# supersimple33/aruco-slam

Measured on AMD Instinct MI355X. Metric: EKF updates/sec at n=1024 landmarks, m=32 obs/frame, higher is better.
Workload: dtype f32 covariance / f64 state

## Files before the change

aruco_slam_amd/csrc/ekf_api.hip:

```cpp
#include <atomic>
#include <cstring>

#include "ekf_host.h"
#include "ekf_kernels.h"

thread_local std::string g_err;

namespace {

std::atomic<ekf_filter*> g_pipelining{nullptr};

void release_pipelining_token(ekf_filter* f) { (void)g_pipelining.compare_exchange_strong(f, nullptr); }

constexpr int kStageSlots = 64;
constexpr int kMacroSuper = 8;
constexpr int kMacroMinTiles = 3000;
constexpr int kTimedKernels = 4;
constexpr int kWideVisible = 1024;
inline int visible_cap(int model) { return model == EKF_MODEL_ROTATIONS ? 50 : 64; }
inline bool wide_frame(int model, int m) { return m > visible_cap(model); }
constexpr int kEventPool = 2048;

struct Layout {
    int64_t cap;
// ... 39 lines not shown
    L.has_cov2 = c.cov_kernel != EKF_COVK_VALU && (c.flags & 5) == 0;
    L.off_cov2 = L.has_cov2 ? w.take((size_t)L.cap * L.cap * L.elem) : 0;
    L.off_wdbg = w.take((size_t)L.kmax * L.cap * 8);
    L.off_idx = w.take((size_t)c.max_visible * 4);
    L.off_z = w.take((size_t)c.max_visible * 7 * 8);
    L.off_status = w.take(256);
    L.off_stamps = w.take(64 * 8);
    L.off_dx = w.take((size_t)L.cap * 8);
    L.off_diag = w.take((size_t)L.cap * 8);
    L.off_xyz = w.take((size_t)256 * 6 * 8);
    L.off_unc = w.take((size_t)256 * 10 * 8);
    {
        const size_t nb = (size_t)L.kmax / EKF_RB;
        L.xl_dop = nb * (nb - 1) / 2 * 256 + 64;
        L.xl_y = L.xl_dop + nb * 256;
        L.xl_jac = L.xl_y + L.kmax;
        L.xl_tag = L.xl_jac + (size_t)L.kmax * EKF_JLD;
        L.xl_xs = L.xl_tag + 32;
        L.xl_xr = L.xl_xs + nb * (nb + 1) / 2 * 256;
        L.xl_stag = L.xl_xr + (size_t)round_up(L.kmax, 16);
        L.xl_len = L.xl_stag + 256;
        L.off_xl = w.take(2 * L.xl_len * 8);
        L.off_done = w.take(256);
        L.off_sync = w.take(256);
        L.wsup_ld = (int)round_up(EKF_CAM + (int64_t)L.lmd * c.max_visible, 32);
        L.off_wsup = w.take((size_t)2 * L.kmax * L.wsup_ld * L.elem);
    }
    {
        const int tmax = (int)(L.cap / 128);
        L.tiles_cap = (L.elem == 4 && c.cov_kernel != EKF_COVK_VALU && c.cov_kernel != EKF_COVK_MFMA_TILE)
                          ? tmax * (tmax + 1) / 2 + 8 * kMacroSuper * kMacroSuper : 0;
        L.off_tiles = w.take((size_t)L.tiles_cap * 4);
    }
    L.off_wwork = wide ? w.take((size_t)L.kmax * L.cap * 8) : 0;
    L.off_xinv = wide ? w.take((size_t)EKF_WIDE_BLOCK * EKF_WIDE_BLOCK * 8) : 0;
    L.total = w.end;
    L.slot_bytes = std::max(align256((size_t)c.max_visible * 4) + align256((size_t)c.max_visible * 56),
                            align256(256 * 48) + align256(256 * 80));
    return L;
}

int check_config(const ekf_config* c) {
    if (!c) return fail(EKF_ERR_INVALID, "config is NULL");
    if (c->max_landmarks < 1) return fail(EKF_ERR_INVALID, "max_landmarks must be >= 1");
    if (c->model != EKF_MODEL_EKF && c->model != EKF_MODEL_ROTATIONS)
        return fail(EKF_ERR_INVALID, "unknown model");
    if (c->max_visible < 1 || c->max_visible > ((c->flags & EKF_FLAG_WIDE_FRAMES) ? kWideVisible : visible_cap(c->model)))
// ... 29 lines not shown
};

struct ekf_filter {
    ekf_config cfg{};
    Layout lay{};
    hipStream_t stream = nullptr;
    hipStream_t big = nullptr;
    hipEvent_t ev_front = nullptr;
    GetterShortcut shortcut;
    int device = 0;
    void* cov = nullptr;
    int64_t ld = 0;
    double* state = nullptr;
    char* ws = nullptr;
    bool bound = false, is_reset = false;
    int n_lm = 0;
    int last_m = 0;
    bool debug_w = false;
    bool debug_stamps = false;
    bool debug_stamps_light = false;
    uint64_t fseq = 0;
    uint64_t done_total = 0;
    uint64_t la_base = 0;
    int la_ok = -1;
    int seq_mode = EKF_SEQ_NONE;
    int tiles_T = -1, tiles_grid = 0;
    PinnedBuffer ring, readback, tiles_host;
    int slot = 0;
    hipEvent_t slot_done[kStageSlots] = {};
    bool timing = false;
    bool timing_cov_only = false;
    std::vector<hipEvent_t> ev;
    int ev_frames = 0;
    double t_sum_us[kTimedKernels] = {};
    int64_t t_cnt[kTimedKernels] = {};
    PinnedBuffer log_pin[2];
    hipEvent_t log_pin_done[2] = {};
    int log_pin_turn = 0;
    int64_t log_stats[4] = {};

    int dims() const { return lay.lmd * n_lm + EKF_CAM; }
    template <typename P> P* at(size_t off) const { return reinterpret_cast<P*>(ws + off); }
};

namespace {

// ... 286 lines not shown
}

struct RunFrame {
    const int32_t* idx;
    const double* z;
    int m;
    double* traj_row;
};

template <class FrameAt>
int run_pipelined(ekf_filter* f, int frames, FrameAt frame_at, void* other) {
    const Layout& L = f->lay;
    int rc = ensure_tiles(f);
    if (rc) return rc;
    void* wbuf[2] = {f->at<void>(L.off_wpanel), f->at<void>(L.off_wpanel2)};
    void* cbuf[2] = {f->cov, other};
    char* wsup0 = f->at<char>(L.off_wsup);
    void* wsup[2] = {wsup0, wsup0 + (size_t)L.kmax * L.wsup_ld * L.elem};
    unsigned long long* sync = f->at<unsigned long long>(L.off_sync);
    int32_t* status = f->at<int32_t>(L.off_status);
    const uint64_t base = f->la_base;
    f->shortcut.run();
    RunFrame nx = frame_at(0);
    for (int t = 0; t < frames; ++t) {
        const int par = t & 1;
        const RunFrame cf_t = nx;
        EkfFrame fr = make_frame(f, cf_t.idx, cf_t.z, cf_t.m, cf_t.traj_row);
        fr.cov = cbuf[0];
        fr.wpanel = wbuf[par];
        if (t > 0) {
            fr.cov = cbuf[par ^ 1];
            fr.wprev = wbuf[par ^ 1];
            fr.wsup_prev = wsup[par ^ 1];
        }
        const int nb = fr.kpad / EKF_RB;
        const int grid = nb * (nb + 1) / 2 + 2 + fr.ncols / 64;
        fr.wsup_ld = L.wsup_ld;
        fr.la_sync = sync;
        fr.la_signal = (t > 0) ? base + (uint64_t)t : 0;
        fr.la_gate = (t > 0) ? base + (uint64_t)t : 0;
        fr.lds_min = grid <= 100 ? 148 * 1024 : 0;
        if (t + 1 < frames) {
            nx = frame_at(t + 1);
            fr.next_idx = nx.idx;
            fr.next_m = nx.m;
            fr.wsup = wsup[par];
        }
        bind_exchange(f, fr);
        by_cov_type(f, [&](auto elem) { ekf_launch_front<decltype(elem)>(fr, f->stream); });
        EkfFrame cu = fr;
        cu.cov = cbuf[par];
        cu.cov_out = cbuf[par ^ 1];
        if (t + 1 < frames) {
            ekf_launch_gate(sync, base + (uint64_t)t + 1, status, f->big);
            by_cov_type(f, [&](auto elem) { ekf_launch_cov_update<decltype(elem)>(cu, 2, f->big); });
            ekf_launch_signal(sync + 1, base + (uint64_t)t + 1, f->big);
        } else {
            by_cov_type(f, [&](auto elem) { ekf_launch_cov_update<decltype(elem)>(cu, 2, f->stream); });
        }
        HIP_TRY(hipGetLastError());
        f->last_m = cf_t.m;
    }
    f->cov = cbuf[frames & 1];
    f->la_base = base + (uint64_t)frames;
    return EKF_OK;
}

struct RunPlan {
    std::vector<char> candidate;
    std::vector<char> joins;
    bool want_runs = false;
};

template <class MOf, class NNewOf>
RunPlan plan_runs(const ekf_filter* f, int frames, MOf m_of, NNewOf nnew_of) {
    RunPlan p;
    p.candidate.assign((size_t)frames, 0);
    p.joins.assign((size_t)frames, 0);
    int prev_kpad = -1;
// ... 70 lines not shown
}

int open_handle(ekf_filter* f) {
    int rc = reserve_host_buffers(f, f->lay);
    if (rc) return rc;
    HIP_TRY(hipStreamCreateWithFlags(&f->big, hipStreamNonBlocking));
    HIP_TRY(hipEventCreateWithFlags(&f->ev_front, hipEventDisableTiming));
    for (hipEvent_t& e : f->slot_done) HIP_TRY(hipEventCreateWithFlags(&e, hipEventDisableTiming));
    return EKF_OK;
}

int clear_buffers(const ekf_filter* f, void* cov, double* state, char* ws, const Layout& L) {
    HIP_TRY(hipMemsetAsync(cov, 0, (size_t)L.cap * L.cap * L.elem, f->stream));
    HIP_TRY(hipMemsetAsync(state, 0, (size_t)L.cap * 8, f->stream));
    HIP_TRY(hipMemsetAsync(ws, 0, L.total, f->stream));
    HIP_TRY(hipMemsetD32Async(reinterpret_cast<hipDeviceptr_t>(ws + L.off_xl), (int)0xFFFBADC0u, L.xl_len * 4, f->stream));
    return EKF_OK;
}

void restart_workspace(ekf_filter* f) {
    f->fseq = 0;
    f->done_total = 0;
    f->la_base = 0;
    f->tiles_T = -1;
    std::memset(f->readback.get(), 0, 256 + (size_t)f->lay.cap * 8);
}

}

extern "C" {

const char* ekf_last_error_string(void) { return g_err.c_str(); }

int ekf_default_config(ekf_config* cfg) {
    if (!cfg) return fail(EKF_ERR_INVALID, "config is NULL");
    std::memset(cfg, 0, sizeof(*cfg));
    cfg->max_landmarks = 50;
    cfg->max_visible = 50;
    cfg->cov_dtype = EKF_COV_F64;
    cfg->quat_mode = EKF_QUAT_AS_WRITTEN;
    cfg->cov_kernel = EKF_COVK_AUTO;
    cfg->model = EKF_MODEL_EKF;
    cfg->initial_camera_uncertainty = 0.1;
    cfg->initial_landmark_uncertainty = 0.7;
    cfg->r_uncertainty = 0.9;
    cfg->q_cam = 0.3;
// ... 603 lines not shown
```

aruco_slam_amd/csrc/ekf_cov_macro.hip:

```cpp
#include <hip/hip_ext.h>
#include "ekf_kernels.h"

typedef float cm_f32x16 __attribute__((ext_vector_type(16)));
typedef float cm_f4 __attribute__((ext_vector_type(4)));

#define CM_NW 8
#define CM_T (64 * CM_NW)
#define CM_LD 132
#define CM_KC 16
#define CM_NBUF 5
#define CM_LDS_BYTES (CM_NBUF * 2 * CM_KC * 128 * 4)

#define CM_MID 0
#define CM_STAGGER 24000

__device__ __forceinline__ void cm_store16(float* p, const cm_f4& v) {
    asm volatile("global_store_dwordx4 %0, %1, off sc1\n\ts_nop 1" ::"v"(p), "v"(v) : "memory");
}

__device__ __forceinline__ void cm_dma16(const float* g, float* lds_wave_base) {
    __builtin_amdgcn_global_load_lds((const __attribute__((address_space(1))) void*)g,
                                     (__attribute__((address_space(3))) void*)lds_wave_base, 16, 0, 0);
}

// ... 13 lines not shown
        if (ch == target) seen = true;
    }
    for (int i = 0; i < steps; ++i) {
        if (i + depth < nch) {
            if (seen) n += dpw;
            if (i + depth == target) seen = true;
        }
        if (i < npb && seen) n += 16;
    }
    return n;
}
template <int N> __device__ __forceinline__ void cm_wait_vm() { asm volatile("s_waitcnt vmcnt(%0)" ::"n"(N) : "memory"); }

template <int KB, int NW>
__global__ __launch_bounds__(64 * NW) __attribute__((amdgpu_waves_per_eu(NW / 2, NW / 2)))
void ekf_cov_update_macro_f32(EkfFrame fr, const uint32_t* __restrict__ tiles) {
    extern __shared__ __attribute__((aligned(16))) float cm_sm[];
    constexpr int NT = 64 * NW, WC = NW / 2, CW = 128 / WC, TJ = CW / 32;
    constexpr int DPW = 16 / NW;
    constexpr int NPB = 2 * TJ;
    constexpr int DEPTH = CM_NBUF - 1;
    static_assert(NW == 8, "wait counts below are worked out for 8 waves");
    const uint32_t tl = tiles[blockIdx.x];
    if (tl == 0xFFFFFFFFu) return;
    const int I = (int)(tl >> 16), J = (int)(tl & 0xFFFFu);
    const int tid = threadIdx.x, lane = tid & 63, l31 = lane & 31, lhi = lane >> 5;
    const int wave = __builtin_amdgcn_readfirstlane(tid >> 6);
    const int wr = wave / WC, wc = wave % WC;
    const int i0 = 128 * I, j0 = 128 * J;
    const float* __restrict__ wp = static_cast<const float*>(fr.wpanel);
    const float* __restrict__ P = static_cast<const float*>(fr.cov);
    float* Pout = fr.cov_out ? static_cast<float*>(fr.cov_out) : static_cast<float*>(fr.cov);
    const int ld = (int)fr.ld, ldw = (int)fr.ldw;
    constexpr int NCH = KB;

    if (blockIdx.x < 512 && ((__builtin_amdgcn_s_getreg((31 << 11) | 4) / (NW / 4)) & 1)) {
        const long long t0 = __builtin_amdgcn_s_memtime();
        while (__builtin_amdgcn_s_memtime() - t0 < CM_STAGGER) __builtin_amdgcn_s_sleep(32);
    }
    const unsigned wlane = (unsigned)(lhi * ldw + 4 * l31);
    auto stage = [&](int c) {
        float* buf = cm_sm + (c % CM_NBUF) * (2 * CM_KC * 128);
        const int rloc = 2 * wave;
        const float* src = wp + (int64_t)(CM_KC * c + rloc) * ldw;
        cm_dma16(src + i0 + wlane, buf + rloc * 128);
        cm_dma16(src + j0 + wlane, buf + CM_KC * 128 + rloc * 128);
    };
// ... 107 lines not shown
        for (int it = 0; it < NPASS; ++it) cm_store16(ob + (int64_t)(RPP * it) * ld + (unsigned)(prow * ld + pcol), rowv[it]);
    }
    if (!dtile) __syncthreads();
    if (!dtile) {
#pragma unroll
    for (int ti = 0; ti < 2; ++ti)
#pragma unroll
        for (int tj = 0; tj < TJ; ++tj)
#pragma unroll
            for (int rg = 0; rg < 4; ++rg) {
                const cm_f4 v = {acc[ti][tj][4 * rg], acc[ti][tj][4 * rg + 1], acc[ti][tj][4 * rg + 2], acc[ti][tj][4 * rg + 3]};
                *reinterpret_cast<cm_f4*>(img + (CW * wc + 32 * tj + l31) * CM_LD + 64 * wr + 32 * ti + 8 * rg + 4 * lhi) = v;
            }
    __syncthreads();
    {
        cm_f4 rowv[NPASS];
#pragma unroll
        for (int it = 0; it < NPASS; ++it) rowv[it] = *reinterpret_cast<const cm_f4*>(img + (RPP * it + prow) * CM_LD + pcol);
        float* ob = Pout + (int64_t)j0 * ld + i0;
#pragma unroll
        for (int it = 0; it < NPASS; ++it) cm_store16(ob + (int64_t)(RPP * it) * ld + (unsigned)(prow * ld + pcol), rowv[it]);
    }
    }
}

int ekf_cov_macro_table(int T, int S, uint32_t* out, int capacity) {
    struct Sup { int si, sj, count; };
    const int NS = (T + S - 1) / S;
    Sup sup[4096];
    int nsup = 0;
    for (int si = 0; si < NS; ++si)
        for (int sj = 0; sj <= si; ++sj) {
            int cnt = 0;
            for (int I = si * S; I < T && I < (si + 1) * S; ++I)
                for (int J = sj * S; J < T && J < (sj + 1) * S && J <= I; ++J) ++cnt;
            if (cnt > 0 && nsup < 4096) sup[nsup++] = Sup{si, sj, cnt};
        }
    for (int a = 1; a < nsup; ++a) {
        const Sup x = sup[a];
        int b = a - 1;
        while (b >= 0 && sup[b].count < x.count) { sup[b + 1] = sup[b]; --b; }
        sup[b + 1] = x;
    }
    int load[8] = {0, 0, 0, 0, 0, 0, 0, 0};
    int owner[4096];
    for (int a = 0; a < nsup; ++a) {
        int x = 0;
        for (int q = 1; q < 8; ++q)
            if (load[q] < load[x]) x = q;
        owner[a] = x;
        load[x] += sup[a].count;
    }
    int maxlen = 0;
    for (int q = 0; q < 8; ++q) maxlen = load[q] > maxlen ? load[q] : maxlen;
    const int grid = 8 * maxlen;
    if (!out) return grid;
    if (grid > capacity) return -1;
    for (int b = 0; b < grid; ++b) out[b] = 0xFFFFFFFFu;
    int pos[8] = {0, 0, 0, 0, 0, 0, 0, 0};
    for (int a = 0; a < nsup; ++a) {
        const int x = owner[a];
        for (int I = sup[a].si * S; I < T && I < (sup[a].si + 1) * S; ++I)
            for (int J = sup[a].sj * S; J < T && J < (sup[a].sj + 1) * S && J <= I; ++J)
                out[8 * (pos[x]++) + x] = ((uint32_t)I << 16) | (uint32_t)J;
    }
    return grid;
}

template <int KB>
static void cm_go(const EkfFrame& fr, hipStream_t s, hipEvent_t e0, hipEvent_t e1) {
    static bool once = false;
    if (!once) {
        (void)hipFuncSetAttribute(reinterpret_cast<const void*>(&ekf_cov_update_macro_f32<KB, CM_NW>),
                                  hipFuncAttributeMaxDynamicSharedMemorySize, CM_LDS_BYTES);
        once = true;
    }
    if (e0) hipExtLaunchKernelGGL((ekf_cov_update_macro_f32<KB, CM_NW>), dim3(fr.cov_grid), dim3(CM_T), CM_LDS_BYTES, s, e0, e1, 0, fr, fr.cov_tiles);
    else hipLaunchKernelGGL((ekf_cov_update_macro_f32<KB, CM_NW>), dim3(fr.cov_grid), dim3(CM_T), CM_LDS_BYTES, s, fr, fr.cov_tiles);
}

void ekf_launch_cov_update_macro(const EkfFrame& fr, hipStream_t s, hipEvent_t e0, hipEvent_t e1) {
    switch (fr.kpad / 16) {
#define CM_CASE(KB) case KB: return cm_go<KB>(fr, s, e0, e1);
        CM_CASE(1) CM_CASE(2) CM_CASE(3) CM_CASE(4) CM_CASE(5) CM_CASE(6) CM_CASE(7) CM_CASE(8) CM_CASE(9) CM_CASE(10)
        CM_CASE(11) CM_CASE(12) CM_CASE(13) CM_CASE(14) CM_CASE(15) CM_CASE(16) CM_CASE(17) CM_CASE(18) CM_CASE(19)
        CM_CASE(20) CM_CASE(21) CM_CASE(22) CM_CASE(23) CM_CASE(24)
#undef CM_CASE
        default: return;
    }
}
```

aruco_slam_amd/csrc/ekf_cov_update.hip:

```cpp
#include <hip/hip_ext.h>
#include "ekf_kernels.h"

template <typename T>
__device__ __forceinline__ void ekf_cov_store(T* p, T v) {
    __hip_atomic_store(p, v, __ATOMIC_RELAXED, __HIP_MEMORY_SCOPE_AGENT);
}

typedef float f32x16 __attribute__((ext_vector_type(16)));
typedef double f64x4 __attribute__((ext_vector_type(4)));

template <typename T>
__global__ __launch_bounds__(256) void ekf_cov_update_valu(EkfFrame fr) {
    __shared__ T sa[16][64];
    __shared__ T sb[16][64];
    const int tid = threadIdx.x, tx = tid & 15, ty = tid >> 4;
    const int i0 = blockIdx.y * 64, j0 = blockIdx.x * 64;
    const T* __restrict__ wp = static_cast<const T*>(fr.wpanel);
    T acc[4][4];
#pragma unroll
    for (int x = 0; x < 4; ++x)
#pragma unroll
        for (int y = 0; y < 4; ++y) acc[x][y] = (T)0;
    for (int kc = 0; kc < fr.kpad; kc += 16) {
#pragma unroll
// ... 19 lines not shown
    }
    T* __restrict__ P = static_cast<T*>(fr.cov);
#pragma unroll
    for (int x = 0; x < 4; ++x) {
        const int row = i0 + ty * 4 + x;
#pragma unroll
        for (int y = 0; y < 4; ++y) {
            const int col = j0 + tx * 4 + y;
            T v = P[(int64_t)row * fr.ld + col];
            if (row == col) v += (T)ekf_qdiag(row, fr.dims, fr.nz);
            P[(int64_t)row * fr.ld + col] = v + acc[x][y];
        }
    }
}

__device__ __forceinline__ void ekf_tri_decode(int item, int& I, int& J) {
    int i = (int)((sqrtf(8.0f * (float)item + 1.0f) - 1.0f) * 0.5f);
    while (i * (i + 1) / 2 > item) --i;
    while ((i + 1) * (i + 2) / 2 <= item) ++i;
    I = i;
    J = item - i * (i + 1) / 2;
}

template <int KB, int DMAX = 3, int WPE = 5>
__global__ __launch_bounds__(256) __attribute__((amdgpu_waves_per_eu(WPE, WPE)))
void ekf_cov_update_mfma_f32(EkfFrame fr, int nitems) {
    __shared__ float tr[4][32][33];
    const int wave = threadIdx.x >> 6, lane = threadIdx.x & 63;
    const int l31 = lane & 31, lhi = lane >> 5;
    const int item = __builtin_amdgcn_readfirstlane(blockIdx.x * 4 + wave);
    if (item >= nitems) return;
    int I, J;
    ekf_tri_decode(item, I, J);
    const int i0 = 32 * I, j0 = 32 * J;
    const float* __restrict__ wp = static_cast<const float*>(fr.wpanel);
    const float* __restrict__ P = static_cast<const float*>(fr.cov);
    float* Pout = fr.cov_out ? static_cast<float*>(fr.cov_out) : static_cast<float*>(fr.cov);
    const int ld = (int)fr.ld, ldw = (int)fr.ldw;
    constexpr int NCH = KB, D = (NCH < DMAX) ? NCH : DMAX;
    float ra[D][8], rb[D][8], pt[16];
    const unsigned wlane = 4u * (unsigned)(lhi * ldw + l31);
    const unsigned plane = 4u * (unsigned)(4 * lhi * ld + l31);
    const uint64_t kstep = 8ull * (uint64_t)ldw;
    uint64_t ua = reinterpret_cast<uint64_t>(wp + i0), ub = reinterpret_cast<uint64_t>(wp + j0);
    const float* __restrict__ ptile = P + (int64_t)i0 * ld + j0;
    float* otile = Pout + (int64_t)i0 * ld + j0;
#define EKF_GLD(dst, voff, sbase) asm volatile("global_load_dword %0, %1, %2" : "=v"(dst) : "v"(voff), "s"(sbase) : "memory")
#define EKF_WAIT16(n, A, B)                                                                              \
    asm volatile("s_waitcnt vmcnt(%16)"                                                                   \
                 : "+v"(A[0]), "+v"(A[1]), "+v"(A[2]), "+v"(A[3]), "+v"(A[4]), "+v"(A[5]), "+v"(A[6]), "+v"(A[7]), \
// ... 29 lines not shown
            case 0: EKF_WAIT16(0, ra[c % D], rb[c % D]); break;
            case 16: EKF_WAIT16(16, ra[c % D], rb[c % D]); break;
            case 32: EKF_WAIT16(32, ra[c % D], rb[c % D]); break;
            case 48: EKF_WAIT16(48, ra[c % D], rb[c % D]); break;
            default: EKF_WAIT16(63, ra[c % D], rb[c % D]); break;
        }
#pragma unroll
        for (int u = 0; u < 8; ++u)
            acc = __builtin_amdgcn_mfma_f32_32x32x2f32(-ra[c % D][u], rb[c % D][u], acc, 0, 0, 0);
        __builtin_amdgcn_sched_barrier(0);
        if (c + D < NCH) {
#pragma unroll
            for (int u = 0; u < 8; ++u) {
                EKF_GLD(ra[c % D][u], wlane, ua);
                EKF_GLD(rb[c % D][u], wlane, ub);
                ua += kstep;
                ub += kstep;
            }
        }
        __builtin_amdgcn_sched_barrier(0);
    }
    asm volatile("s_waitcnt vmcnt(0)"
                 : "+v"(pt[0]), "+v"(pt[1]), "+v"(pt[2]), "+v"(pt[3]), "+v"(pt[4]), "+v"(pt[5]), "+v"(pt[6]), "+v"(pt[7]),
                   "+v"(pt[8]), "+v"(pt[9]), "+v"(pt[10]), "+v"(pt[11]), "+v"(pt[12]), "+v"(pt[13]), "+v"(pt[14]), "+v"(pt[15]));
#undef EKF_GLD
#undef EKF_WAIT16
    const float qlane = (I == J) ? (float)ekf_qdiag(i0 + l31, fr.dims, fr.nz) : 0.0f;
    float out[16];
    auto stf = [](float* base, unsigned off, float v) { ekf_cov_store(reinterpret_cast<float*>(reinterpret_cast<char*>(base) + off), v); };
#pragma unroll
    for (int reg = 0; reg < 16; ++reg) {
        const int rl = (reg & 3) + 8 * (reg >> 2) + 4 * lhi;
        const float v = (pt[reg] + ((rl == l31) ? qlane : 0.0f)) + acc[reg];
        out[reg] = v;
        stf(otile + (int64_t)((reg & 3) + 8 * (reg >> 2)) * ld, plane, v);
    }
    if (I != J) {
#pragma unroll
        for (int reg = 0; reg < 16; ++reg)
            tr[wave][(reg & 3) + 8 * (reg >> 2) + 4 * lhi][l31] = out[reg];
        __builtin_amdgcn_wave_barrier();
        float* pm = Pout + (int64_t)j0 * ld + i0;
        const unsigned mlane = 4u * (unsigned)(lhi * ld + l31);
#pragma unroll
        for (int it = 0; it < 16; ++it)
            stf(pm + (int64_t)(2 * it) * ld, mlane, tr[wave][l31][2 * it + lhi]);
    }
}

__global__ __launch_bounds__(256) void ekf_cov_update_mfma_f64(EkfFrame fr, int nitems) {
    __shared__ double tr[4][32][33];
    const int wave = threadIdx.x >> 6, lane = threadIdx.x & 63;
    const int c = lane & 15, g = lane >> 4;
    const int item = blockIdx.x * 4 + wave;
    if (item >= nitems) return;
    int I, J;
    ekf_tri_decode(item, I, J);
    const int i0 = 32 * I, j0 = 32 * J;
    const double* __restrict__ wp = static_cast<const double*>(fr.wpanel);
    const double* P = static_cast<const double*>(fr.cov);
    double* Pout = fr.cov_out ? static_cast<double*>(fr.cov_out) : static_cast<double*>(fr.cov);
    const int64_t ld = fr.ld, ldw = fr.ldw;

    double pt[2][2][4];
#pragma unroll
    for (int ri = 0; ri < 2; ++ri)
#pragma unroll
        for (int ci = 0; ci < 2; ++ci)
#pragma unroll
            for (int r = 0; r < 4; ++r)
                pt[ri][ci][r] = P[(int64_t)(i0 + 16 * ri + g + 4 * r) * ld + j0 + 16 * ci + c];
    f64x4 acc[2][2];
#pragma unroll
    for (int ri = 0; ri < 2; ++ri)
// ... 15 lines not shown
            b1[u] = wb[off + 16];
        }
#pragma unroll
        for (int u = 0; u < 4; ++u) {
            acc[0][0] = __builtin_amdgcn_mfma_f64_16x16x4f64(-a0[u], b0[u], acc[0][0], 0, 0, 0);
            acc[0][1] = __builtin_amdgcn_mfma_f64_16x16x4f64(-a0[u], b1[u], acc[0][1], 0, 0, 0);
            acc[1][0] = __builtin_amdgcn_mfma_f64_16x16x4f64(-a1[u], b0[u], acc[1][0], 0, 0, 0);
            acc[1][1] = __builtin_amdgcn_mfma_f64_16x16x4f64(-a1[u], b1[u], acc[1][1], 0, 0, 0);
        }
    }
#pragma unroll
    for (int ri = 0; ri < 2; ++ri)
#pragma unroll
        for (int ci = 0; ci < 2; ++ci)
#pragma unroll
            for (int r = 0; r < 4; ++r) {
                const int rl = 16 * ri + g + 4 * r, cl = 16 * ci + c;
                double v = pt[ri][ci][r];
                if (I == J && rl == cl) v += ekf_qdiag(i0 + rl, fr.dims, fr.nz);
                v += acc[ri][ci][r];
                ekf_cov_store(Pout + (int64_t)(i0 + rl) * ld + j0 + cl, v);
                if (I != J) tr[wave][rl][cl] = v;
            }
    if (I != J) {
        __builtin_amdgcn_wave_barrier();
        const int l31 = lane & 31, lhi = lane >> 5;
#pragma unroll
        for (int it = 0; it < 16; ++it) {
            const int cc = 2 * it + lhi;
            ekf_cov_store(Pout + (int64_t)(j0 + cc) * ld + i0 + l31, tr[wave][l31][cc]);
        }
    }
}

__global__ __launch_bounds__(256) void ekf_cov_update_mfma_f64_split(EkfFrame fr, int nitems) {
    __shared__ double tr[32][33];
    const int wave = threadIdx.x >> 6, lane = threadIdx.x & 63;
    const int c = lane & 15, g = lane >> 4;
    const int ri = wave >> 1, ci = wave & 1;
    int I, J;
    ekf_tri_decode(blockIdx.x, I, J);
    const int i0 = 32 * I, j0 = 32 * J;
    const double* __restrict__ wp = static_cast<const double*>(fr.wpanel);
    const double* P = static_cast<const double*>(fr.cov);
    double* Pout = fr.cov_out ? static_cast<double*>(fr.cov_out) : static_cast<double*>(fr.cov);
    const int64_t ld = fr.ld, ldw = fr.ldw;
    double pt[4];
#pragma unroll
    for (int r = 0; r < 4; ++r) pt[r] = P[(int64_t)(i0 + 16 * ri + g + 4 * r) * ld + j0 + 16 * ci + c];
    f64x4 acc = {0.0, 0.0, 0.0, 0.0};
    const double* wa = wp + (int64_t)g * ldw + i0 + 16 * ri + c;
    const double* wb = wp + (int64_t)g * ldw + j0 + 16 * ci + c;
    const int steps = fr.kpad >> 2;
    for (int ks = 0; ks < steps; ks += 4) {
        double a[4], b[4];
#pragma unroll
        for (int u = 0; u < 4; ++u) {
            const int64_t off = (int64_t)(4 * (ks + u)) * ldw;
            a[u] = wa[off];
            b[u] = wb[off];
        }
#pragma unroll
        for (int u = 0; u < 4; ++u) acc = __builtin_amdgcn_mfma_f64_16x16x4f64(-a[u], b[u], acc, 0, 0, 0);
    }
#pragma unroll
    for (int r = 0; r < 4; ++r) {
        const int rl = 16 * ri + g + 4 * r, cl = 16 * ci + c;
        double v = pt[r];
        if (I == J && rl == cl) v += ekf_qdiag(i0 + rl, fr.dims, fr.nz);
        v += acc[r];
        ekf_cov_store(Pout + (int64_t)(i0 + rl) * ld + j0 + cl, v);
        if (I != J) tr[rl][cl] = v;
    }
    if (I != J) {
        __syncthreads();
        const int l31 = threadIdx.x & 31;
        for (int cc = threadIdx.x >> 5; cc < 32; cc += 8)
            ekf_cov_store(Pout + (int64_t)(j0 + cc) * ld + i0 + l31, tr[l31][cc]);
    }
}

__global__ void ekf_gate_kernel(unsigned long long* counter, unsigned long long target, int32_t* status, int max_polls) {
    if (threadIdx.x != 0) return;
    int it = 0;
    while (__hip_atomic_load(counter, __ATOMIC_RELAXED, __HIP_MEMORY_SCOPE_SYSTEM) < target) {
        if (++it > max_polls) { atomicOr(status, EKF_ST_GATE_TIMEOUT); break; }
        __builtin_amdgcn_s_sleep(8);
    }
}
__global__ void ekf_signal_kernel(unsigned long long* counter, unsigned long long value) {
    if (threadIdx.x == 0) __hip_atomic_store(counter, value, __ATOMIC_RELAXED, __HIP_MEMORY_SCOPE_SYSTEM);
}
void ekf_launch_gate(unsigned long long* counter, unsigned long long target, int32_t* status, hipStream_t s, int max_polls) {
    hipLaunchKernelGGL(ekf_gate_kernel, dim3(1), dim3(64), 0, s, counter, target, status, max_polls);
}
void ekf_launch_signal(unsigned long long* counter, unsigned long long value, hipStream_t s) {
    hipLaunchKernelGGL(ekf_signal_kernel, dim3(1), dim3(64), 0, s, counter, value);
}

#define EKF_COV_LAUNCH(kernel, grid, block, s, e0, e1, ...)                                     \
    do {                                                                                         \
        if (e0) hipExtLaunchKernelGGL(kernel, grid, block, 0, s, e0, e1, 0, __VA_ARGS__);        \
        else hipLaunchKernelGGL(kernel, grid, block, 0, s, __VA_ARGS__);                         \
    } while (0)

static inline int ekf_tri_items(const EkfFrame& fr) {
    const int t = (fr.dims + 31) / 32;
    return t * (t + 1) / 2;
}

template <>
void ekf_launch_cov_update<float>(const EkfFrame& fr, int variant, hipStream_t s, hipEvent_t e0, hipEvent_t e1) {
    if (variant == 1) {
        EKF_COV_LAUNCH(ekf_cov_update_valu<float>, dim3(fr.ncols / 64, fr.ncols / 64), dim3(256), s, e0, e1, fr);
    } else if (fr.cov_tiles) {
        ekf_launch_cov_update_macro(fr, s, e0, e1);
    } else {
        const int items = ekf_tri_items(fr);
        const dim3 grid((items + 3) / 4), block(256);
        switch (fr.kpad / 16) {
#define EKF_COV_CASE(KB) case KB: EKF_COV_LAUNCH((ekf_cov_update_mfma_f32<KB, 3, (KB <= 8) ? 5 : 4>), grid, block, s, e0, e1, fr, items); break;
            EKF_COV_CASE(1) EKF_COV_CASE(2) EKF_COV_CASE(3) EKF_COV_CASE(4) EKF_COV_CASE(5) EKF_COV_CASE(6)
            EKF_COV_CASE(7) EKF_COV_CASE(8) EKF_COV_CASE(9) EKF_COV_CASE(10) EKF_COV_CASE(11) EKF_COV_CASE(12)
            EKF_COV_CASE(13) EKF_COV_CASE(14) EKF_COV_CASE(15) EKF_COV_CASE(16) EKF_COV_CASE(17) EKF_COV_CASE(18)
            EKF_COV_CASE(19) EKF_COV_CASE(20) EKF_COV_CASE(21) EKF_COV_CASE(22) EKF_COV_CASE(23) EKF_COV_CASE(24)
            default: break;
#undef EKF_COV_CASE
        }
    }
}
template <>
void ekf_launch_cov_update<double>(const EkfFrame& fr, int variant, hipStream_t s, hipEvent_t e0, hipEvent_t e1) {
    if (variant == 1) {
        EKF_COV_LAUNCH(ekf_cov_update_valu<double>, dim3(fr.ncols / 64, fr.ncols / 64), dim3(256), s, e0, e1, fr);
    } else {
        const int items = ekf_tri_items(fr);
        if (items <= 2048)
            EKF_COV_LAUNCH(ekf_cov_update_mfma_f64_split, dim3(items), dim3(256), s, e0, e1, fr, items);
        else
            EKF_COV_LAUNCH(ekf_cov_update_mfma_f64, dim3((items + 3) / 4), dim3(256), s, e0, e1, fr, items);
    }
}
```

aruco_slam_amd/csrc/ekf_front_impl.h:

```cpp
#pragma once
#include "ekf_solve_big.h"

#define FR_T 512
#define FR_ALD 66
#define FR_KS 96
#define FR_KS64 48
__host__ __device__ inline size_t fr_chunk_a_len(int kpad, bool fix, int elem) {
    const size_t a = (size_t)kpad * FR_ALD;
    const size_t st = elem == 4 ? (size_t)(FR_KS * 128 + FR_KS * 64 + 128 * 64) / 2 : (size_t)(2 * FR_KS64 * 64 + 64 * 64);
    return (fix && a < st) ? st : a;
}
#define FR_SLOTS 4

typedef double pf64x4 __attribute__((ext_vector_type(4)));
template <typename T>
__device__ __forceinline__ void fr_w_store(T* p, T v) {
    __hip_atomic_store(p, v, __ATOMIC_RELAXED, __HIP_MEMORY_SCOPE_AGENT);
}
typedef float fr_f32x16 __attribute__((ext_vector_type(16)));

__device__ __forceinline__ void ekf_poll_sleep() { __builtin_amdgcn_s_sleep(4); }

template <int MODEL>
__device__ __forceinline__ void fr_measure(const EkfFrame& fr, const double* cam, const int* lmc, double* hs,
// ... 212 lines not shown
    int* lmc = reinterpret_cast<int*>(rsd + fr.kpad);
    const int tid = threadIdx.x;
    if (fr.stamps && !fr.stamps_heavy && tid == 0) fr.stamps[16 + ((long long)fr.seqno & 15)] = wall_clock64();
    if (fr.la_signal && tid == 0)
        __hip_atomic_store(fr.la_sync, fr.la_signal, __ATOMIC_RELAXED, __HIP_MEMORY_SCOPE_SYSTEM);
    double cam[EKF_CAM];
#pragma unroll
    for (int a = 0; a < EKF_CAM; ++a) cam[a] = fr.state[a];
    if (tid < fr.m) lmc[tid] = ekf_lm_column(fr, LMD, tid, true);
    __syncthreads();
    fr_measure<MODEL>(fr, cam, lmc, hs, rsd, tid, true);
    __syncthreads();
    double* __restrict__ xj = fr.xl + fr.xl_jac;
    const int nel = fr.k * JC;
    for (int e = tid; e < nel; e += FR_T) ekf_stc(xj + e, hs[e]);
    for (int e = tid; e < fr.kpad; e += FR_T) ekf_stc(fr.xr + e, rsd[e]);
    if (tid == 0) {
        ekf_stc(fr.xl + fr.xl_tag, fr.seqno);
        ekf_stc(fr.xl + fr.xl_tag + 16, fr.seqno);
    }
    if (fr.stamps && tid == 0) fr.stamps[55] = wall_clock64();
    if (fr.la_gate && tid == 0) {
        int it = 0;
        while (__hip_atomic_load(fr.la_sync + 1, __ATOMIC_RELAXED, __HIP_MEMORY_SCOPE_SYSTEM) < fr.la_gate) {
            if (++it > (1 << 22)) { ekf_raise(fr, EKF_ST_GATE_TIMEOUT); break; }
            __builtin_amdgcn_s_sleep(8);
        }
    }
}

__device__ __forceinline__ int fr_tag_stale(double tag, double seqno) { return !ekf_is_sent(tag) && tag != seqno; }
struct SvIoFused {
    const EkfFrame& fr;
    int spin_fail, stale;
    __device__ __forceinline__ bool settled(const sf64x4& v) const {
        return !__any(ekf_is_sent(v[0]) || ekf_is_sent(v[1]) || ekf_is_sent(v[2]) || ekf_is_sent(v[3]));
    }
    __device__ __forceinline__ void settle_block(sf64x4& v, int i, int tc, int lane) {
        const double* base = fr.xs + sv_blk_index(i, tc);
        int it = 0;
        while (!settled(v)) {
            if (++it > EKF_SPIN_MAX) { spin_fail = 1; break; }
            ekf_poll_sleep();
            v = sf64x4{ekf_ldc(base + 2 * lane), ekf_ldc(base + 2 * lane + 1), ekf_ldc(base + 128 + 2 * lane),
                       ekf_ldc(base + 129 + 2 * lane)};
        }
    }
    __device__ __forceinline__ sf64x4 fetch_resid(int tc, int g) {
        const double* base = fr.xr + EKF_RB * tc + g;
        sf64x4 v = {ekf_ldc(base), ekf_ldc(base + 4), ekf_ldc(base + 8), ekf_ldc(base + 12)};
        int it = 0;
// ... 864 lines not shown
```

aruco_slam_amd/csrc/ekf_kernels.h:

```cpp
#pragma once
#include <hip/hip_runtime.h>
#include <stdint.h>
#include "ekf_device.h"

#define EKF_ST_NOT_SPD 1
#define EKF_ST_TIMEOUT 4
#define EKF_ST_STALE_JAC 16
#define EKF_ST_STALE_COL 32
#define EKF_ST_STALE_S 64
#define EKF_ST_BAD_INDEX 128
#define EKF_ST_GATE_TIMEOUT 256

struct EkfFrame {
    void* cov;
    int64_t ld;
    double* state;
    int32_t model;
    int32_t dims;
    int32_t ncols;
    int32_t m;
    int32_t k;
    int32_t kpad;
    const int32_t* idx;
    const double* z;
// ... 5 lines not shown
    double* sblk;
    int32_t sblk_rows;
    double* lmat;
    int32_t ldl;
    double* dinv;
    double* lop;
    double* dop;
    double* yvec;
    void* wpanel;
    int64_t ldw;
    double* wdbg;
    int32_t* status;
    double* traj_row;
    double* dxvec;
    long long* stamps;
    int32_t stamps_heavy;
    const int32_t* next_idx;
    int32_t next_m;
    void* cov_out;
    const void* wprev;
    const void* wsup_prev;
    unsigned long long* la_sync;
    unsigned long long la_signal, la_gate;
    int32_t lds_min;
    void* wsup;
    int32_t wsup_ld;
    EkfNoise nz;
    int32_t quat_mode;
    double* xl;
    double* xl_next;
    int32_t xl_dop, xl_y, xl_jac;
    int32_t xl_len;
    double* xs;
    double* xr;
    double* xs_tag;
    int32_t n_lm;
    unsigned long long* done_ctr;
    unsigned long long done_target;
    int32_t xl_tag;
    double seqno;
    double* state_host;
    int32_t* status_host;
    const uint32_t* cov_tiles;
    int32_t cov_grid;
};

__device__ __forceinline__ void ekf_raise(const EkfFrame& fr, int bits) {
    atomicOr(fr.status, bits);
    if (fr.status_host) __hip_atomic_store(fr.status_host, 1, __ATOMIC_RELAXED, __HIP_MEMORY_SCOPE_SYSTEM);
}

__device__ __forceinline__ int ekf_lm_column(const EkfFrame& fr, int lmd, int j, bool flag) {
    int i = fr.idx[j];
    if ((unsigned)i >= (unsigned)fr.n_lm) {
        if (flag) ekf_raise(fr, EKF_ST_BAD_INDEX);
        i = 0;
    }
    return EKF_CAM + lmd * i;
}

__device__ inline void ekf_inject_camera(const EkfFrame& fr, const double err[3], const double x[3]) {
    double q[4] = {fr.state[3], fr.state[4], fr.state[5], fr.state[6]};
    ekf_quat_inject(q, err, fr.quat_mode);
    for (int i = 0; i < 4; ++i) fr.state[3 + i] = q[i];
    for (int i = 0; i < 3; ++i) fr.state[7 + i] = 0.0;
    if (fr.traj_row) {
        fr.traj_row[0] = x[0]; fr.traj_row[1] = x[1]; fr.traj_row[2] = x[2];
        for (int i = 0; i < 4; ++i) fr.traj_row[3 + i] = q[i];
    }
}

template <typename T> void ekf_launch_front(const EkfFrame& fr, hipStream_t s);
template <typename T> void ekf_launch_gather(const EkfFrame& fr, hipStream_t s);
void ekf_launch_solve(const EkfFrame& fr, hipStream_t s);
template <typename T> void ekf_launch_panel(const EkfFrame& fr, hipStream_t s);
template <typename T> void ekf_launch_cov_update(const EkfFrame& fr, int variant, hipStream_t s,
                                                 hipEvent_t e0 = nullptr, hipEvent_t e1 = nullptr);
void ekf_launch_cov_update_macro(const EkfFrame& fr, hipStream_t s, hipEvent_t e0 = nullptr, hipEvent_t e1 = nullptr);
int ekf_cov_macro_table(int T, int S, uint32_t* out, int capacity);
void ekf_launch_gate(unsigned long long* counter, unsigned long long target, int32_t* status, hipStream_t s,
                     int max_polls = 1 << 22);
void ekf_launch_signal(unsigned long long* counter, unsigned long long value, hipStream_t s);

#define EKF_WIDE_REUSE_ROWS 384
#define EKF_WIDE_BLOCK 64
template <typename T> void ekf_launch_wide_front(const EkfFrame& fr, double* aw, int rp, hipStream_t s);
void ekf_launch_wide_factor(const EkfFrame& fr, double* aw, double* xinv, int rp, hipStream_t s);
template <typename T> void ekf_launch_wide_finish(const EkfFrame& fr, const double* aw, hipStream_t s);

template <typename T>
void ekf_launch_add_markers(void* cov, int64_t ld, double* state, int32_t dims,
                            const double* xyz_dev, const double* unc_dev, double default_unc,
                            int32_t count, hipStream_t s);
void ekf_launch_inject_rot(const EkfFrame& fr, int n_lm, hipStream_t s);
template <typename T>
void ekf_launch_add_markers_rot(void* cov, int64_t ld, double* state, int32_t dims, const double* pose6_dev,
                                const double* unc_dev, double default_unc, int32_t count, hipStream_t s);
void ekf_launch_log_prepare(const double* poses_dev, int64_t count, int rd, double* z_dev, hipStream_t s);
template <typename T>
void ekf_launch_log_add_markers(int model, void* cov, int64_t ld, double* state, int32_t dims, const double* poses_dev,
                                const int32_t* slots_dev, double default_unc, int32_t count, hipStream_t s);
// ... 33 lines not shown
```

Before: 42630.

## Signal per-block covariance completion and mirror only rows the next frame reads

Replaces the separate signal kernel after the covariance update with per-block atomic arrivals on sharded counters. The next frame's front kernel now polls the summed count against the number of launched blocks, so it can start as soon as the last tile finishes rather than after an extra launch. In the non-macro MFMA paths, the mirrored lower-triangle stores are also limited to rows touched by the frame after next (via that frame's landmark indices), cutting write traffic. This adds atomics and a barrier per block, and leaves the skipped mirror rows stale on the assumption that later frames never read them.

```diff
diff --git a/aruco_slam_amd/csrc/ekf_api.hip b/aruco_slam_amd/csrc/ekf_api.hip
--- a/aruco_slam_amd/csrc/ekf_api.hip
+++ b/aruco_slam_amd/csrc/ekf_api.hip
@@ -85,7 +85,7 @@
         L.xl_len = L.xl_stag + 256;
         L.off_xl = w.take(2 * L.xl_len * 8);
         L.off_done = w.take(256);
-        L.off_sync = w.take(256);
+        L.off_sync = w.take(256 + EKF_DONE_SHARDS * 128);
         L.wsup_ld = (int)round_up(EKF_CAM + (int64_t)L.lmd * c.max_visible, 32);
         L.off_wsup = w.take((size_t)2 * L.kmax * L.wsup_ld * L.elem);
     }
@@ -161,6 +161,7 @@
     uint64_t fseq = 0;
     uint64_t done_total = 0;
     uint64_t la_base = 0;
+    uint64_t la_arrived = 0;
     int la_ok = -1;
     int seq_mode = EKF_SEQ_NONE;
     int tiles_T = -1, tiles_grid = 0;
@@ -493,6 +494,7 @@
     const uint64_t base = f->la_base;
     f->shortcut.run();
     RunFrame nx = frame_at(0);
+    uint64_t gate_next = 0;
     for (int t = 0; t < frames; ++t) {
         const int par = t & 1;
         const RunFrame cf_t = nx;
@@ -509,7 +511,7 @@
         fr.wsup_ld = L.wsup_ld;
         fr.la_sync = sync;
         fr.la_signal = (t > 0) ? base + (uint64_t)t : 0;
-        fr.la_gate = (t > 0) ? base + (uint64_t)t : 0;
+        fr.la_gate = (t > 0) ? gate_next : 0;
         fr.lds_min = grid <= 100 ? 148 * 1024 : 0;
         if (t + 1 < frames) {
             nx = frame_at(t + 1);
@@ -523,9 +525,16 @@
         cu.cov = cbuf[par];
         cu.cov_out = cbuf[par ^ 1];
         if (t + 1 < frames) {
+            cu.cov_done = sync;
+            cu.mirror_sel = 1;
+            if (t + 2 < frames) {
+                const RunFrame r2 = frame_at(t + 2);
+                cu.mirror_idx = r2.idx;
+                cu.mirror_m = r2.m;
+            }
             ekf_launch_gate(sync, base + (uint64_t)t + 1, status, f->big);
-            by_cov_type(f, [&](auto elem) { ekf_launch_cov_update<decltype(elem)>(cu, 2, f->big); });
-            ekf_launch_signal(sync + 1, base + (uint64_t)t + 1, f->big);
+            f->la_arrived += (uint64_t)by_cov_type(f, [&](auto elem) { return ekf_launch_cov_update<decltype(elem)>(cu, 2, f->big); });
+            gate_next = f->la_arrived;
         } else {
             by_cov_type(f, [&](auto elem) { ekf_launch_cov_update<decltype(elem)>(cu, 2, f->stream); });
         }
@@ -642,6 +651,7 @@
     f->fseq = 0;
     f->done_total = 0;
     f->la_base = 0;
+    f->la_arrived = 0;
     f->tiles_T = -1;
     std::memset(f->readback.get(), 0, 256 + (size_t)f->lay.cap * 8);
 }
diff --git a/aruco_slam_amd/csrc/ekf_cov_macro.hip b/aruco_slam_amd/csrc/ekf_cov_macro.hip
--- a/aruco_slam_amd/csrc/ekf_cov_macro.hip
+++ b/aruco_slam_amd/csrc/ekf_cov_macro.hip
@@ -59,7 +59,12 @@
     constexpr int DEPTH = CM_NBUF - 1;
     static_assert(NW == 8, "wait counts below are worked out for 8 waves");
     const uint32_t tl = tiles[blockIdx.x];
-    if (tl == 0xFFFFFFFFu) return;
+    if (tl == 0xFFFFFFFFu) {
+        if (fr.cov_done && threadIdx.x == 0)
+            __hip_atomic_fetch_add(fr.cov_done + EKF_DONE_OFF + EKF_DONE_STRIDE * (blockIdx.x & (EKF_DONE_SHARDS - 1)), 1ull,
+                                   __ATOMIC_RELAXED, __HIP_MEMORY_SCOPE_AGENT);
+        return;
+    }
     const int I = (int)(tl >> 16), J = (int)(tl & 0xFFFFu);
     const int tid = threadIdx.x, lane = tid & 63, l31 = lane & 31, lhi = lane >> 5;
     const int wave = __builtin_amdgcn_readfirstlane(tid >> 6);
@@ -213,6 +218,7 @@
         for (int it = 0; it < NPASS; ++it) cm_store16(ob + (int64_t)(RPP * it) * ld + (unsigned)(prow * ld + pcol), rowv[it]);
     }
     }
+    if (fr.cov_done) ekf_cov_arrive(fr.cov_done);
 }
 
 int ekf_cov_macro_table(int T, int S, uint32_t* out, int capacity) {
@@ -259,7 +265,7 @@
 }
 
 template <int KB>
-static void cm_go(const EkfFrame& fr, hipStream_t s, hipEvent_t e0, hipEvent_t e1) {
+static int cm_go(const EkfFrame& fr, hipStream_t s, hipEvent_t e0, hipEvent_t e1) {
     static bool once = false;
     if (!once) {
         (void)hipFuncSetAttribute(reinterpret_cast<const void*>(&ekf_cov_update_macro_f32<KB, CM_NW>),
@@ -268,15 +274,16 @@
     }
     if (e0) hipExtLaunchKernelGGL((ekf_cov_update_macro_f32<KB, CM_NW>), dim3(fr.cov_grid), dim3(CM_T), CM_LDS_BYTES, s, e0, e1, 0, fr, fr.cov_tiles);
     else hipLaunchKernelGGL((ekf_cov_update_macro_f32<KB, CM_NW>), dim3(fr.cov_grid), dim3(CM_T), CM_LDS_BYTES, s, fr, fr.cov_tiles);
-}
-
-void ekf_launch_cov_update_macro(const EkfFrame& fr, hipStream_t s, hipEvent_t e0, hipEvent_t e1) {
+    return fr.cov_grid;
+}
+
+int ekf_launch_cov_update_macro(const EkfFrame& fr, hipStream_t s, hipEvent_t e0, hipEvent_t e1) {
     switch (fr.kpad / 16) {
 #define CM_CASE(KB) case KB: return cm_go<KB>(fr, s, e0, e1);
         CM_CASE(1) CM_CASE(2) CM_CASE(3) CM_CASE(4) CM_CASE(5) CM_CASE(6) CM_CASE(7) CM_CASE(8) CM_CASE(9) CM_CASE(10)
         CM_CASE(11) CM_CASE(12) CM_CASE(13) CM_CASE(14) CM_CASE(15) CM_CASE(16) CM_CASE(17) CM_CASE(18) CM_CASE(19)
         CM_CASE(20) CM_CASE(21) CM_CASE(22) CM_CASE(23) CM_CASE(24)
 #undef CM_CASE
-        default: return;
-    }
-}
+        default: return 0;
+    }
+}
diff --git a/aruco_slam_amd/csrc/ekf_cov_update.hip b/aruco_slam_amd/csrc/ekf_cov_update.hip
--- a/aruco_slam_amd/csrc/ekf_cov_update.hip
+++ b/aruco_slam_amd/csrc/ekf_cov_update.hip
@@ -65,10 +65,8 @@
     J = item - i * (i + 1) / 2;
 }
 
-template <int KB, int DMAX = 3, int WPE = 5>
-__global__ __launch_bounds__(256) __attribute__((amdgpu_waves_per_eu(WPE, WPE)))
-void ekf_cov_update_mfma_f32(EkfFrame fr, int nitems) {
-    __shared__ float tr[4][32][33];
+template <int KB, int DMAX>
+__device__ __forceinline__ void ekf_cov_tile_mfma_f32(const EkfFrame& fr, int nitems, float (*tr)[32][33]) {
     const int wave = threadIdx.x >> 6, lane = threadIdx.x & 63;
     const int l31 = lane & 31, lhi = lane >> 5;
     const int item = __builtin_amdgcn_readfirstlane(blockIdx.x * 4 + wave);
@@ -144,7 +142,8 @@
     }
     asm volatile("s_waitcnt vmcnt(0)"
                  : "+v"(pt[0]), "+v"(pt[1]), "+v"(pt[2]), "+v"(pt[3]), "+v"(pt[4]), "+v"(pt[5]), "+v"(pt[6]), "+v"(pt[7]),
-                   "+v"(pt[8]), "+v"(pt[9]), "+v"(pt[10]), "+v"(pt[11]), "+v"(pt[12]), "+v"(pt[13]), "+v"(pt[14]), "+v"(pt[15]));
+                   "+v"(pt[8]), "+v"(pt[9]), "+v"(pt[10]), "+v"(pt[11]), "+v"(pt[12]), "+v"(pt[13]), "+v"(pt[14]), "+v"(pt[15])
+                 :: "memory");
 #undef EKF_GLD
 #undef EKF_WAIT16
     const float qlane = (I == J) ? (float)ekf_qdiag(i0 + l31, fr.dims, fr.nz) : 0.0f;
@@ -157,21 +156,35 @@
         out[reg] = v;
         stf(otile + (int64_t)((reg & 3) + 8 * (reg >> 2)) * ld, plane, v);
     }
-    if (I != J) {
+    const uint32_t rows = (I != J) ? ekf_mirror_rows(fr, j0) : 0u;
+    if (rows) {
 #pragma unroll
         for (int reg = 0; reg < 16; ++reg)
             tr[wave][(reg & 3) + 8 * (reg >> 2) + 4 * lhi][l31] = out[reg];
         __builtin_amdgcn_wave_barrier();
         float* pm = Pout + (int64_t)j0 * ld + i0;
         const unsigned mlane = 4u * (unsigned)(lhi * ld + l31);
+        float mv[16];
+#pragma unroll
+        for (int it = 0; it < 16; ++it) mv[it] = tr[wave][l31][2 * it + lhi];
+        asm volatile(""
+                     : "+v"(mv[0]), "+v"(mv[1]), "+v"(mv[2]), "+v"(mv[3]), "+v"(mv[4]), "+v"(mv[5]), "+v"(mv[6]), "+v"(mv[7]),
+                       "+v"(mv[8]), "+v"(mv[9]), "+v"(mv[10]), "+v"(mv[11]), "+v"(mv[12]), "+v"(mv[13]), "+v"(mv[14]), "+v"(mv[15]));
 #pragma unroll
         for (int it = 0; it < 16; ++it)
-            stf(pm + (int64_t)(2 * it) * ld, mlane, tr[wave][l31][2 * it + lhi]);
-    }
-}
-
-__global__ __launch_bounds__(256) void ekf_cov_update_mfma_f64(EkfFrame fr, int nitems) {
-    __shared__ double tr[4][32][33];
+            if ((rows >> (2 * it + lhi)) & 1u) stf(pm + (int64_t)(2 * it) * ld, mlane, mv[it]);
+    }
+}
+
+template <int KB, int DMAX = 3, int WPE = 5>
+__global__ __launch_bounds__(256) __attribute__((amdgpu_waves_per_eu(WPE, WPE)))
+void ekf_cov_update_mfma_f32(EkfFrame fr, int nitems) {
+    __shared__ float tr[4][32][33];
+    ekf_cov_tile_mfma_f32<KB, DMAX>(fr, nitems, tr);
+    if (fr.cov_done) ekf_cov_arrive(fr.cov_done);
+}
+
+__device__ __forceinline__ void ekf_cov_tile_mfma_f64(const EkfFrame& fr, int nitems, double (*tr)[32][33]) {
     const int wave = threadIdx.x >> 6, lane = threadIdx.x & 63;
     const int c = lane & 15, g = lane >> 4;
     const int item = blockIdx.x * 4 + wave;
@@ -233,15 +246,22 @@
                 ekf_cov_store(Pout + (int64_t)(i0 + rl) * ld + j0 + cl, v);
                 if (I != J) tr[wave][rl][cl] = v;
             }
-    if (I != J) {
+    const uint32_t rows = (I != J) ? ekf_mirror_rows(fr, j0) : 0u;
+    if (rows) {
         __builtin_amdgcn_wave_barrier();
         const int l31 = lane & 31, lhi = lane >> 5;
 #pragma unroll
         for (int it = 0; it < 16; ++it) {
             const int cc = 2 * it + lhi;
-            ekf_cov_store(Pout + (int64_t)(j0 + cc) * ld + i0 + l31, tr[wave][l31][cc]);
-        }
-    }
+            if ((rows >> cc) & 1u) ekf_cov_store(Pout + (int64_t)(j0 + cc) * ld + i0 + l31, tr[wave][l31][cc]);
+        }
+    }
+}
+
+__global__ __launch_bounds__(256) void ekf_cov_update_mfma_f64(EkfFrame fr, int nitems) {
+    __shared__ double tr[4][32][33];
+    ekf_cov_tile_mfma_f64(fr, nitems, tr);
+    if (fr.cov_done) ekf_cov_arrive(fr.cov_done);
 }
 
 __global__ __launch_bounds__(256) void ekf_cov_update_mfma_f64_split(EkfFrame fr, int nitems) {
@@ -283,12 +303,14 @@
         ekf_cov_store(Pout + (int64_t)(i0 + rl) * ld + j0 + cl, v);
         if (I != J) tr[rl][cl] = v;
     }
-    if (I != J) {
+    const uint32_t rows = (I != J) ? ekf_mirror_rows(fr, j0) : 0u;
+    if (rows) {
         __syncthreads();
         const int l31 = threadIdx.x & 31;
         for (int cc = threadIdx.x >> 5; cc < 32; cc += 8)
-            ekf_cov_store(Pout + (int64_t)(j0 + cc) * ld + i0 + l31, tr[l31][cc]);
-    }
+            if ((rows >> cc) & 1u) ekf_cov_store(Pout + (int64_t)(j0 + cc) * ld + i0 + l31, tr[l31][cc]);
+    }
+    if (fr.cov_done) ekf_cov_arrive(fr.cov_done);
 }
 
 __global__ void ekf_gate_kernel(unsigned long long* counter, unsigned long long target, int32_t* status, int max_polls) {
@@ -321,11 +343,12 @@
 }
 
 template <>
-void ekf_launch_cov_update<float>(const EkfFrame& fr, int variant, hipStream_t s, hipEvent_t e0, hipEvent_t e1) {
+int ekf_launch_cov_update<float>(const EkfFrame& fr, int variant, hipStream_t s, hipEvent_t e0, hipEvent_t e1) {
     if (variant == 1) {
         EKF_COV_LAUNCH(ekf_cov_update_valu<float>, dim3(fr.ncols / 64, fr.ncols / 64), dim3(256), s, e0, e1, fr);
+        return (fr.ncols / 64) * (fr.ncols / 64);
     } else if (fr.cov_tiles) {
-        ekf_launch_cov_update_macro(fr, s, e0, e1);
+        return ekf_launch_cov_update_macro(fr, s, e0, e1);
     } else {
         const int items = ekf_tri_items(fr);
         const dim3 grid((items + 3) / 4), block(256);
@@ -338,17 +361,20 @@
             default: break;
 #undef EKF_COV_CASE
         }
+        return (int)grid.x;
     }
 }
 template <>
-void ekf_launch_cov_update<double>(const EkfFrame& fr, int variant, hipStream_t s, hipEvent_t e0, hipEvent_t e1) {
+int ekf_launch_cov_update<double>(const EkfFrame& fr, int variant, hipStream_t s, hipEvent_t e0, hipEvent_t e1) {
     if (variant == 1) {
         EKF_COV_LAUNCH(ekf_cov_update_valu<double>, dim3(fr.ncols / 64, fr.ncols / 64), dim3(256), s, e0, e1, fr);
-    } else {
-        const int items = ekf_tri_items(fr);
-        if (items <= 2048)
-            EKF_COV_LAUNCH(ekf_cov_update_mfma_f64_split, dim3(items), dim3(256), s, e0, e1, fr, items);
-        else
-            EKF_COV_LAUNCH(ekf_cov_update_mfma_f64, dim3((items + 3) / 4), dim3(256), s, e0, e1, fr, items);
-    }
-}
+        return (fr.ncols / 64) * (fr.ncols / 64);
+    }
+    const int items = ekf_tri_items(fr);
+    if (items <= 2048) {
+        EKF_COV_LAUNCH(ekf_cov_update_mfma_f64_split, dim3(items), dim3(256), s, e0, e1, fr, items);
+        return items;
+    }
+    EKF_COV_LAUNCH(ekf_cov_update_mfma_f64, dim3((items + 3) / 4), dim3(256), s, e0, e1, fr, items);
+    return (items + 3) / 4;
+}
diff --git a/aruco_slam_amd/csrc/ekf_front_impl.h b/aruco_slam_amd/csrc/ekf_front_impl.h
--- a/aruco_slam_amd/csrc/ekf_front_impl.h
+++ b/aruco_slam_amd/csrc/ekf_front_impl.h
@@ -258,11 +258,17 @@
     if (fr.stamps && tid == 0) fr.stamps[55] = wall_clock64();
     if (fr.la_gate && tid == 0) {
         int it = 0;
-        while (__hip_atomic_load(fr.la_sync + 1, __ATOMIC_RELAXED, __HIP_MEMORY_SCOPE_SYSTEM) < fr.la_gate) {
+        for (;;) {
+            unsigned long long arrived = 0;
+#pragma unroll
+            for (int x = 0; x < EKF_DONE_SHARDS; ++x)
+                arrived += __hip_atomic_load(fr.la_sync + EKF_DONE_OFF + EKF_DONE_STRIDE * x, __ATOMIC_RELAXED, __HIP_MEMORY_SCOPE_SYSTEM);
+            if (arrived >= fr.la_gate) break;
             if (++it > (1 << 22)) { ekf_raise(fr, EKF_ST_GATE_TIMEOUT); break; }
             __builtin_amdgcn_s_sleep(8);
         }
     }
+    if (fr.stamps && tid == 0) fr.stamps[56] = wall_clock64();
 }
 
 __device__ __forceinline__ int fr_tag_stale(double tag, double seqno) { return !ekf_is_sent(tag) && tag != seqno; }
diff --git a/aruco_slam_amd/csrc/ekf_kernels.h b/aruco_slam_amd/csrc/ekf_kernels.h
--- a/aruco_slam_amd/csrc/ekf_kernels.h
+++ b/aruco_slam_amd/csrc/ekf_kernels.h
@@ -51,6 +51,9 @@
     const void* wsup_prev;
     unsigned long long* la_sync;
     unsigned long long la_signal, la_gate;
+    unsigned long long* cov_done;
+    const int32_t* mirror_idx;
+    int32_t mirror_m, mirror_sel;
     int32_t lds_min;
     void* wsup;
     int32_t wsup_ld;
@@ -73,6 +76,35 @@
     const uint32_t* cov_tiles;
     int32_t cov_grid;
 };
+
+#define EKF_DONE_SHARDS 8
+#define EKF_DONE_STRIDE 16
+#define EKF_DONE_OFF 32
+
+__device__ __forceinline__ void ekf_cov_arrive(unsigned long long* done) {
+    asm volatile("s_waitcnt vmcnt(0)" ::: "memory");
+    __syncthreads();
+    if (threadIdx.x == 0) {
+        __hip_atomic_fetch_add(done + EKF_DONE_OFF + EKF_DONE_STRIDE * (blockIdx.x & (EKF_DONE_SHARDS - 1)), 1ull,
+                               __ATOMIC_RELAXED, __HIP_MEMORY_SCOPE_AGENT);
+    }
+}
+
+__device__ __forceinline__ uint32_t ekf_mirror_rows(const EkfFrame& fr, int j0) {
+    if (!fr.mirror_sel) return 0xFFFFFFFFu;
+    const int lmd = fr.model == 1 ? EkfModel<1>::LMD : EkfModel<0>::LMD;
+    const uint64_t span = (1ull << lmd) - 1;
+    uint32_t bits = (j0 == 0 && fr.mirror_m > 0) ? (1u << EKF_CAM) - 1 : 0u;
+    for (int d = (int)(threadIdx.x & 63); d < fr.mirror_m; d += 64) {
+        int i = fr.mirror_idx[d];
+        if ((unsigned)i >= (unsigned)fr.n_lm) i = 0;
+        const int r = EKF_CAM + lmd * i - j0;
+        if (r > -lmd && r < 32) bits |= (uint32_t)(r >= 0 ? span << r : span >> -r);
+    }
+#pragma unroll
+    for (int o = 32; o > 0; o >>= 1) bits |= (uint32_t)__shfl_xor((int)bits, o);
+    return __builtin_amdgcn_readfirstlane(bits);
+}
 
 __device__ __forceinline__ void ekf_raise(const EkfFrame& fr, int bits) {
     atomicOr(fr.status, bits);
@@ -103,9 +135,9 @@
 template <typename T> void ekf_launch_gather(const EkfFrame& fr, hipStream_t s);
 void ekf_launch_solve(const EkfFrame& fr, hipStream_t s);
 template <typename T> void ekf_launch_panel(const EkfFrame& fr, hipStream_t s);
-template <typename T> void ekf_launch_cov_update(const EkfFrame& fr, int variant, hipStream_t s,
-                                                 hipEvent_t e0 = nullptr, hipEvent_t e1 = nullptr);
-void ekf_launch_cov_update_macro(const EkfFrame& fr, hipStream_t s, hipEvent_t e0 = nullptr, hipEvent_t e1 = nullptr);
+template <typename T> int ekf_launch_cov_update(const EkfFrame& fr, int variant, hipStream_t s,
+                                                hipEvent_t e0 = nullptr, hipEvent_t e1 = nullptr);
+int ekf_launch_cov_update_macro(const EkfFrame& fr, hipStream_t s, hipEvent_t e0 = nullptr, hipEvent_t e1 = nullptr);
 int ekf_cov_macro_table(int T, int S, uint32_t* out, int capacity);
 void ekf_launch_gate(unsigned long long* counter, unsigned long long target, int32_t* status, hipStream_t s,
                      int max_polls = 1 << 22);
```

New measurement: 42840, median of 6. About the same (+0.5%).
